# ChenJiahao031008/EAO-Fusion

Hardware: AMD Instinct MI355X
Metric: ORB kpts/s (640x480, 1k feat) + local-BA residuals/s (20 KF x 3k pts) (higher is better)
Workload: dtype u8; 1 GPU; ORBextractor FAST+rBRIEF, 640x480, 8-level pyramid, nFeatures 1000, batch=64 synthetic frames per GPU (BASELINE configs[1]); parallelism=frames sharded per GPU, no data-path collective

## Files before the change

### eao_fusion_amd/csrc/orb.hip

```cpp
#include "orb_internal.h"

using namespace eao::orb;

namespace {

__constant__ __align__(16) signed char c_pattern[1024] = {
#include "orb_pattern.inc"
};

constexpr int kResizeRows = 4;
__device__ __forceinline__ unsigned udot2w(unsigned a, unsigned b) {
    typedef unsigned short us2 __attribute__((ext_vector_type(2)));
    return __builtin_amdgcn_udot2(__builtin_bit_cast(us2, a), __builtin_bit_cast(us2, b), 0u, false);
}

struct ResizeLevel { int w, h, pitch, off; };
struct ResizeArgs {
    ResizeLevel D, S;
    double invX, invY;
    int srcIsInput;
    int pyrFrameBytes;
    int G;
    float invG;
    int frameAffinity;
// ... 985 lines not shown
    const float minZ = A.mb, minD = -3, maxD = A.mbf / minZ;
    const float minU = uL - maxD, maxU = uL - minD;
    float outU = -1.0f, outD = -1.0f;
    int outS = -1;
    if (!(maxU < 0)) {
        const uint4 a0 = A.dl[2 * iL], a1 = A.dl[2 * iL + 1];
        unsigned best = 0xFFFFFFFFu;
        for (int iR = lane; iR < A.nr; iR += 64) {
            const eao_keypoint kr = A.kr[iR];
            const float r = 2.0f * A.scale[kr.octave];
            const int maxr = (int)ceilf(kr.y + r), minr = (int)floorf(kr.y - r);
            if (row < minr || row > maxr) continue;
            if (kr.octave < levelL - 1 || kr.octave > levelL + 1) continue;
            if (!(kr.x >= minU && kr.x <= maxU)) continue;
            const uint4 b0 = A.dr[2 * iR], b1 = A.dr[2 * iR + 1];
            const unsigned d = __popc(a0.x ^ b0.x) + __popc(a0.y ^ b0.y) + __popc(a0.z ^ b0.z) + __popc(a0.w ^ b0.w) +
                               __popc(a1.x ^ b1.x) + __popc(a1.y ^ b1.y) + __popc(a1.z ^ b1.z) + __popc(a1.w ^ b1.w);
            best = min(best, (d << 16) | (unsigned)iR);
        }
        for (int dlt = 32; dlt >= 1; dlt >>= 1) best = min(best, (unsigned)__shfl_xor((int)best, dlt));
        const int bestDist = (int)(best >> 16);
        if (best != 0xFFFFFFFFu && bestDist < refc::TH_HIGH) {
            const int bestIdxR = (int)(best & 0xFFFF);
            const float uR0 = A.kr[bestIdxR].x;
            const float sf = A.invScale[levelL];
            const int suL = (int)roundf(uL * sf), svL = (int)roundf(vL * sf), suR0 = (int)roundf(uR0 * sf);
            const int w = 5, Lw = 5;
            int pl, pr;
            const uint8_t* imgL = level_ptr(g, sl, levelL, A.frame, &pl);
            const uint8_t* imgR = level_ptr(g, sr, levelL, A.frame, &pr);
            const int lw = g->L[levelL].w, lh = g->L[levelL].h;
            const float iniu = (float)(suR0 + Lw - w), endu = (float)(suR0 + Lw + w + 1);
            if (!(iniu < 0 || endu >= (float)lw)) {
                const int cL = px_reflect(imgL, pl, lw, lh, suL, svL);
                int dL0 = 0, dL1 = 0, px0x = 0, px0y = 0, px1x = 0, px1y = 0;
                const bool has1 = lane + 64 < 121;
                px0y = lane / 11; px0x = lane - px0y * 11;
                dL0 = px_reflect(imgL, pl, lw, lh, suL - w + px0x, svL - w + px0y) - cL;
                if (has1) {
                    px1y = (lane + 64) / 11; px1x = lane + 64 - px1y * 11;
                    dL1 = px_reflect(imgL, pl, lw, lh, suL - w + px1x, svL - w + px1y) - cL;
                }
                int dists[11];
                int bestSad = 0x7FFFFFFF, bestinc = 0;
#pragma unroll
                for (int inc = -5; inc <= 5; inc++) {
                    const int cR = px_reflect(imgR, pr, lw, lh, suR0 + inc, svL);
                    int sacc = abs(dL0 - (px_reflect(imgR, pr, lw, lh, suR0 + inc - w + px0x, svL - w + px0y) - cR));
                    if (has1) sacc += abs(dL1 - (px_reflect(imgR, pr, lw, lh, suR0 + inc - w + px1x, svL - w + px1y) - cR));
                    for (int dlt = 32; dlt >= 1; dlt >>= 1) sacc += __shfl_xor(sacc, dlt);
                    dists[inc + 5] = sacc;
                    if (sacc < bestSad) { bestSad = sacc; bestinc = inc; }
                }
                if (!(bestinc == -Lw || bestinc == Lw)) {
                    float dist1 = 0, dist2 = 0, dist3 = 0;
#pragma unroll
                    for (int k = 0; k < 11; k++) {
                        if (k == Lw + bestinc - 1) dist1 = (float)dists[k];
                        if (k == Lw + bestinc) dist2 = (float)dists[k];
                        if (k == Lw + bestinc + 1) dist3 = (float)dists[k];
                    }
                    const float deltaR = (dist1 - dist3) / (2.0f * (dist1 + dist3 - 2.0f * dist2));
                    if (!(deltaR < -1 || deltaR > 1)) {
                        float bestuR = A.scale[levelL] * ((float)suR0 + (float)bestinc + deltaR);
                        float disparity = uL - bestuR;
                        if (disparity >= 0 && disparity < maxD) {
                            if (disparity <= 0) { disparity = 0.01f; bestuR = uL - 0.01f; }
                            outD = A.mbf / disparity;
                            outU = bestuR;
                            outS = bestSad;
                        }
                    }
                }
            }
        }
    }
    if (lane == 0) { A.uRight[iL] = outU; A.depth[iL] = outD; A.sad[iL] = outS; }
}

namespace eao {
namespace orb {

static int blur_mfma_mode() { static const int mode = [] { const char* e = getenv("EAO_ORB_BLUR_MFMA"); return e ? atoi(e) : 1; }(); return mode; }

eao_status enqueue(eao_orb* h, const uint8_t* d_img, int pitch0, long long fs0, int batch, eao_keypoint* d_kps,
                   uint8_t* d_desc, int cap, int* d_n, hipStream_t st) {
    const Geom& g = h->geom;
    eao::Range rAll("eao_orb_extract: enqueue");
    ImgSrc s;
    s.img0 = d_img; s.pitch0 = pitch0; s.fs0 = fs0; s.pyr = h->d_pyr.p;
    h->lastSrc = s; h->lastBatch = batch; h->lastComplete = false; h->pyrFrame = -1;
    const bool prof = h->profiling;
    hipEvent_t* ev = nullptr;
    if (prof) {
        if (h->evUsed + kProfEvents > h->evs.size()) {
            const size_t old = h->evs.size();
            h->evs.resize(old + kProfEvents * 16, nullptr);
            for (size_t i = old; i < h->evs.size(); i++) EAO_HIP(hipEventCreate(&h->evs[i]));
        }
        ev = &h->evs[h->evUsed];
        h->evUsed += kProfEvents;
        EAO_HIP(hipEventRecord(ev[0], st));
    }
    eao_status so;
    if (h->evLastValid && h->lastStream != st) {
        if ((so = order_behind_last_call(h, st))) return so;
    }
    h->lastStream = st;
    EAO_HIP(hipEventRecord(h->evStart, st));
    const hipStream_t ss = h->side;
    const int cells0 = g.L[0].nCells;
    const bool early0 = !prof && g.nlevels > 1 && g.L[0].cellBase == 0 && cells0 < g.totalCells;
    const int aff = (batch & 7) == 0 ? 1 : 0;
    auto fast = [&](hipStream_t str, int first, int end) {
        eao::Range rg("orb: FAST cells");
        const bool whole = first == 0 && end == g.totalCells, narrow = g.fastStride == 48;
        auto* kern = whole ? (narrow ? k_fast_cells<true, 48> : k_fast_cells<true, kTileStrideWide>)
                           : (narrow ? k_fast_cells<false, 48> : k_fast_cells<false, kTileStrideWide>);
        hipLaunchKernelGGL(kern, dim3(128 * ((end - first + 127) / 128), batch), dim3(64), g.fastLdsBytes, str, h->d_geom.p, h->d_cells.p, s,
                           h->d_cellcand.p, h->d_cellcnt.p, 0, first, end, aff);
    };
    const int mid = early0 && batch >= 48 && g.nlevels > 3 ? 3 : 0;
    const bool qtEarly = mid > 0 && batch <= 96;
    const int src0Aligned = ((((uintptr_t)s.img0 | (uintptr_t)s.pitch0 | (uintptr_t)(batch > 1 ? s.fs0 : 0)) & 3) == 0) ? 1 : 0;
    auto quadtree = [&](hipStream_t str, int lFirst, int nLev) {
        eao::Range rg("orb: quad-tree");
        launch_quadtree(h, str, batch, 0, lFirst, nLev);
    };
    auto blur = [&]() -> eao_status {
        EAO_HIP(hipStreamWaitEvent(ss, h->evFork, 0));
        if (prof) EAO_HIP(hipEventRecord(ev[6], ss));
        {
            eao::Range rg("orb: blur");
            if (g.mTotalTiles && blur_mfma_mode())
                hipLaunchKernelGGL(k_blur7_mfma, dim3(g.mTotalTiles, batch), dim3(256), 0, ss, h->d_geom.p, s, h->d_blur.p, h->d_blurTab.p, 0, src0Aligned, aff);
            else hipLaunchKernelGGL(k_blur7, dim3(g.totalTiles, batch), dim3(256), 0, ss, h->d_geom.p, s, h->d_blur.p, 0, src0Aligned, aff);
        }
        if (prof) EAO_HIP(hipEventRecord(ev[7], ss));
        EAO_HIP(hipEventRecord(h->evJoin, ss));
        return EAO_OK;
    };
    auto describe = [&](hipStream_t str, int lFirst, int lEnd, int writeN) {
        eao::Range rg("orb: orientation + description");
        int pairs = 0;
        for (int l = lFirst; l < lEnd; l++) pairs += eao::cdiv(g.L[l].listCap, 2);
        const int gx = std::max(1, eao::cdiv(std::min(pairs, eao::cdiv(cap, 2) + g.nlevels), 4));
        hipLaunchKernelGGL(k_orient_describe, aff ? dim3(8 * gx, batch / 8) : dim3(gx, batch), dim3(256), 0, str,
                           h->d_geom.p, s, h->d_blur.p, h->d_levelkps.p, h->d_levelcnt.p, d_kps, d_desc, d_n, cap, 0, g.nlevels, lFirst, lEnd, writeN, aff);
    };
    if (h->pyrFused && batch <= 32) {
        auto pyramid = [&] {
            eao::Range rg("orb: pyramid");
            hipLaunchKernelGGL(k_pyramid_fused, dim3(h->pyr.tilesX * h->pyr.tilesY, 1, batch), dim3(kPyrThreads), h->pyrLds, st, h->pyr, s, 0);
        };
        if (prof) {
            pyramid();
            EAO_HIP(hipEventRecord(ev[1], st));
            EAO_HIP(hipEventRecord(h->evFork, st));
            if ((so = blur())) return so;
            EAO_HIP(hipStreamWaitEvent(st, h->evJoin, 0));
            EAO_HIP(hipEventRecord(ev[9], st));
            fast(st, 0, g.totalCells);
            EAO_HIP(hipEventRecord(ev[2], st));
            quadtree(st, 0, g.nlevels);
            EAO_HIP(hipEventRecord(ev[3], st));
            EAO_HIP(hipEventRecord(ev[4], st));
        } else {
            EAO_HIP(hipStreamWaitEvent(ss, h->evStart, 0));
            fast(ss, 0, cells0);
            quadtree(ss, 0, 1);
            pyramid();
            EAO_HIP(hipEventRecord(h->evFork, st));
            if ((so = blur())) return so;
            fast(st, cells0, g.totalCells);
            quadtree(st, 1, g.nlevels - 1);
            EAO_HIP(hipStreamWaitEvent(st, h->evJoin, 0));
        }
    } else {
        if (early0) {
            EAO_HIP(hipStreamWaitEvent(ss, h->evStart, 0));
            fast(ss, 0, cells0);
        }
        for (int l = 1; l < g.nlevels; l++) {
            const int G4 = eao::cdiv(g.L[l].w, 4);
            ResizeArgs ra;
            ra.G = G4; ra.invG = 1.0f / (float)G4;
            ra.D = {g.L[l].w, g.L[l].h, g.L[l].pitch, g.L[l].off};
            ra.S = {g.L[l - 1].w, g.L[l - 1].h, g.L[l - 1].pitch, g.L[l - 1].off};
            ra.invX = 1. / ((double)g.L[l].w / g.L[l - 1].w); ra.invY = 1. / ((double)g.L[l].h / g.L[l - 1].h);
            ra.srcIsInput = l == 1; ra.pyrFrameBytes = g.pyrFrameBytes;
            ra.frameAffinity = aff;
            { eao::Range rg("orb: pyramid"); hipLaunchKernelGGL(k_resize, dim3(eao::cdiv(G4 * eao::cdiv(g.L[l].h, kResizeRows), 64), 1, batch), dim3(64), 0, st, ra, s, 0); }
            if (l == mid - 1) {
                EAO_HIP(hipEventRecord(h->evMid, st));
                EAO_HIP(hipStreamWaitEvent(ss, h->evMid, 0));
                fast(ss, cells0, g.L[mid].cellBase);
                if (qtEarly) quadtree(ss, 0, mid);
            }
        }
        if (early0 && !qtEarly) EAO_HIP(hipEventRecord(h->evFast0, ss));
        if (prof) {
            EAO_HIP(hipEventRecord(ev[1], st));
            EAO_HIP(hipEventRecord(h->evFork, st));
            if ((so = blur())) return so;
            EAO_HIP(hipStreamWaitEvent(st, h->evJoin, 0));
            EAO_HIP(hipEventRecord(ev[9], st));
            fast(st, 0, g.totalCells);
            EAO_HIP(hipEventRecord(ev[2], st));
        } else {
            EAO_HIP(hipEventRecord(h->evFork, st));
            fast(st, early0 ? (mid ? g.L[mid].cellBase : cells0) : 0, g.totalCells);
            if ((so = blur())) return so;
            if (early0 && !qtEarly) EAO_HIP(hipStreamWaitEvent(st, h->evFast0, 0));
        }
        quadtree(st, qtEarly ? mid : 0, g.nlevels - (qtEarly ? mid : 0));
        if (prof) EAO_HIP(hipEventRecord(ev[3], st));
        EAO_HIP(hipStreamWaitEvent(st, h->evJoin, 0));
        if (prof) EAO_HIP(hipEventRecord(ev[4], st));
    }
    describe(st, 0, g.nlevels, 1);
    if (prof) {
        EAO_HIP(hipEventRecord(ev[5], st));
        EAO_HIP(hipEventRecord(ev[8], st));
    }
    h->evLastValid = true;
    if (h->everyCallEvent) { EAO_HIP(hipEventRecord(h->evLast, st)); h->evLastRecorded = true; }
    EAO_HIP(hipGetLastError());
    return EAO_OK;
}

__global__ __launch_bounds__(256) void k_stream_download(const uint4* __restrict__ src, uint4* __restrict__ dst, size_t n16) {
    for (size_t i = (size_t)blockIdx.x * 256 + threadIdx.x; i < n16; i += (size_t)gridDim.x * 256) dst[i] = src[i];
}

struct PyrExportLevel { int w, h, srcPitch, srcOff, dstPitch, rowChunks, chunkBase; long long dstOff; };
struct PyrExportArgs { int nlevels, border, totalChunks, pyrFrameBytes; PyrExportLevel L[kMaxLevels]; };
__global__ __launch_bounds__(256) void k_pyramid_export(PyrExportArgs A, ImgSrc s, int frame, uint8_t* __restrict__ dst) {
    const int idx = blockIdx.x * 256 + threadIdx.x;
    if (idx >= A.totalChunks) return;
    int l = 0;
    while (l + 1 < A.nlevels && idx >= A.L[l + 1].chunkBase) l++;
    const PyrExportLevel& L = A.L[l];
    const int r = idx - L.chunkBase, row = r / L.rowChunks, ch = r - row * L.rowChunks;
    const uint8_t* src = l == 0 ? s.img0 + (long long)frame * s.fs0 : s.pyr + (long long)frame * A.pyrFrameBytes + L.srcOff;
    const int pitch = l == 0 ? s.pitch0 : L.srcPitch;
    int y = row - A.border;
    y = y < 0 ? -y : (y >= L.h ? 2 * L.h - 2 - y : y);
    y = min(max(y, 0), L.h - 1);
    const uint8_t* srow = src + (long long)y * pitch;
    unsigned w4[4];
#pragma unroll
    for (int q = 0; q < 4; q++) {
        unsigned v = 0;
#pragma unroll
        for (int b = 0; b < 4; b++) {
            int x = ch * 16 + q * 4 + b - A.border;
            x = x < 0 ? -x : (x >= L.w ? 2 * L.w - 2 - x : x);
            x = min(max(x, 0), L.w - 1);
            v |= (unsigned)srow[x] << (8 * b);
        }
        w4[q] = v;
    }
    *reinterpret_cast<uint4*>(dst + L.dstOff + (long long)row * L.dstPitch + ch * 16) = make_uint4(w4[0], w4[1], w4[2], w4[3]);
}

eao_status enqueue_pyramid_export(eao_orb* h, int frame, int border) {
    const Geom& g = h->geom;
    for (int l = 0; l < g.nlevels; l++) EAO_REQUIRE(border < g.L[l].w && border < g.L[l].h, "level %d is smaller than the border", l);
    PyrExportArgs A;
    A.nlevels = g.nlevels; A.border = border; A.pyrFrameBytes = g.pyrFrameBytes;
    size_t off = 0;
    int chunks = 0;
    for (int l = 0; l < g.nlevels; l++) {
        PyrExportLevel& L = A.L[l];
        L.w = g.L[l].w; L.h = g.L[l].h; L.srcPitch = g.L[l].pitch; L.srcOff = g.L[l].off;
// ... 145 lines not shown
```

### eao_fusion_amd/csrc/orb_host.hip

```cpp
#include "orb_internal.h"

using namespace eao::orb;

namespace eao {
namespace orb {

eao_status build_geometry(eao_orb* h, int W, int H) {
    const eao_orb_cfg& c = h->cfg;
    Geom& g = h->geom;
    std::memset(&g, 0, sizeof(g));
    g.nlevels = c.nlevels; g.W = W; g.H = H;
    g.iniTh = c.ini_th_fast; g.minTh = c.min_th_fast;
    for (int i = 0; i < 16; i++) g.umax[i] = h->umax[i];
    h->cells.clear();
    int off = 0, kpBase = 0, candBase = 0, tileBase = 0, maxCell = 0, scanCap = 0, maxList = 0, maxSw = 0, maxSh = 0;
    for (int l = 0; l < c.nlevels; l++) {
        LevelGeom& L = g.L[l];
        const float s = h->invScale[l];
        L.w = cv_round((float)W * s);
        L.h = cv_round((float)H * s);
        EAO_REQUIRE(L.w < 4096 && L.h < 4096, "level %d is %dx%d: coordinates are packed in 12 bits", l, L.w, L.h);
        const int maxBX = L.w - kEdge + 3, maxBY = L.h - kEdge + 3;
        const float width = (float)(maxBX - kMinBorder), height = (float)(maxBY - kMinBorder);
        const int nCols = (int)(width / (float)refc::FAST_CELL), nRows = (int)(height / (float)refc::FAST_CELL);
// ... 111 lines not shown
            }
            coefCap = (coefCap + 7) & ~3;
            P.coefOff = (int)lds; P.coefCap = coefCap;
            lds += (size_t)coefCap * 16;
            h->pyrLds = lds;
            h->pyrFused = lds <= 64 * 1024 && h->cfg.scale_factor <= 2.0f;
            for (int l = 1; l < c.nlevels; l++)
                if (P.L[l].invX > 2.0 || P.L[l].invY > 2.0) h->pyrFused = false;
            if (h->pyrFused) {
                std::vector<int2> cxv, cyv;
                for (int l = 1; l < c.nlevels; l++) {
                    P.L[l].coefXOff = (int)cxv.size(); P.L[l].coefYOff = (int)cyv.size();
                    for (int d = 0; d < g.L[l].w; d++) { int o; unsigned w2; resize_coef_host(d, P.L[l].invX, g.L[l - 1].w, true, &o, &w2); cxv.push_back(make_int2(o, (int)w2)); }
                    for (int d = 0; d < g.L[l].h; d++) { int o; unsigned w2; resize_coef_host(d, P.L[l].invY, g.L[l - 1].h, false, &o, &w2); cyv.push_back(make_int2(o, (int)w2)); }
                }
                eao_status st2 = h->d_pyrRanges.reserve(table.size());
                if (st2) return st2;
                if ((st2 = h->d_pyrCoef.reserve(cxv.size() + cyv.size()))) return st2;
                EAO_HIP(hipMemcpy(h->d_pyrRanges.p, table.data(), table.size() * sizeof(int4), hipMemcpyHostToDevice));
                EAO_HIP(hipMemcpy(h->d_pyrCoef.p, cxv.data(), cxv.size() * sizeof(int2), hipMemcpyHostToDevice));
                EAO_HIP(hipMemcpy(h->d_pyrCoef.p + cxv.size(), cyv.data(), cyv.size() * sizeof(int2), hipMemcpyHostToDevice));
                P.ranges = h->d_pyrRanges.p;
                P.coefX = h->d_pyrCoef.p; P.coefY = h->d_pyrCoef.p + cxv.size();
            }
        }
    }
    g.scanCap = scanCap;
    g.fastMaxTested = std::max(1, (maxSw - 6) * (maxSh - 6));
    g.fastStride = maxSw + 3 <= 48 ? 48 : kTileStrideWide;
    g.fastTileBytes = ((maxSh * g.fastStride) + 15) & ~15;
    g.fastLdsBytes = g.fastTileBytes + ((2 * g.fastMaxTested + 15) & ~15) + ((((maxSw - 4) * (maxSh - 4)) + 15) & ~15) + 64;
    h->quadLds = (size_t)maxList * (2 * sizeof(short4) + sizeof(int) * kQtNodeInts) + (size_t)scanCap * sizeof(int);
    g.qtNodesGlobal = 0; g.qtNodeFrameBytes = 0;
    if (h->quadLds > 100 * 1024) {
        g.qtNodesGlobal = 1;
        long long noff = 0;
        for (int l = 0; l < c.nlevels; l++) {
            g.L[l].nodeOff = noff;
            noff += (long long)align256((size_t)g.L[l].listCap * (2 * sizeof(short4) + sizeof(int) * kQtNodeInts) + (size_t)scanCap * sizeof(int));
        }
        g.qtNodeFrameBytes = noff;
        h->quadLds = 0;
    }
    h->quadLds = (h->quadLds + 15) & ~(size_t)15;
    g.qtKeysOff = (int)h->quadLds;
    const size_t kQtLdsCand = std::min<size_t>(8192, std::max<size_t>(2048, ((size_t)h->cfg.nfeatures * 4 + 63) & ~(size_t)63));
    g.qtLdsCand = (int)std::min<size_t>(kQtLdsCand, h->quadLds < 76 * 1024 ? (76 * 1024 - h->quadLds) / 6 : 0) & ~7;
    h->quadLds += (size_t)g.qtLdsCand * 6;
    if (g.qtNodesGlobal) { g.qtLdsCand = 0; h->quadLds = 0; }
    {
        float cf[7]; double sum = 0;
        for (int i = 0; i < 7; i++) { double x = i - 3; cf[i] = (float)std::exp(-0.5 / 4.0 * x * x); sum += cf[i]; }
        const int expect[7] = {18, 34, 49, 55, 49, 34, 18};
        for (int i = 0; i < 7; i++)
            if (cv_round((double)(float)(cf[i] * (1. / sum)) * 256.0) != expect[i]) { eao::set_error("gaussian taps mismatch"); return EAO_ERR_INTERNAL; }
    }
    {
        std::vector<BlurMLevelIn> in;
        for (int l = 0; l < c.nlevels; l++) in.push_back({g.L[l].w, g.L[l].h, l == 0 ? (g.L[l].w + 3) & ~3 : g.L[l].pitch});
        const BlurMTables T = blur_m_build(in);
        EAO_REQUIRE(T.maxEntry <= 127, "blur table entry %d does not fit int8", T.maxEntry);
        int mBase = 0, any = 0;
        for (int l = 0; l < c.nlevels; l++) {
            LevelGeom& L = g.L[l];
            const BlurMLevel& M = T.level[l];
            L.mOk = M.ok; L.mTilesX = M.tilesX; L.mBlocksY = M.blocksY; L.mXIdx = M.xIdx; L.mYIdx = M.yIdx;
            const int valu = eao::cdiv(L.tilesX * eao::cdiv(L.h, kBlurRows), kBlurStripsPerWg);
            int walkLen;
            const int mfma = eao::cdiv(M.tilesX * blur_m_walks(M.blocksY, &walkLen), 4);
            L.mTileBase = mBase;
            mBase += !M.ok ? valu : l == 0 ? std::max(valu, mfma) : mfma;
            any |= M.ok;
        }
        g.mTotalTiles = any ? mBase : 0;
        g.mFragOff = (int)((T.idx.size() * sizeof(int) + kBlurMFrag - 1) / kBlurMFrag * kBlurMFrag);
        if (any) {
            std::vector<uint8_t> blob((size_t)g.mFragOff + T.frag.size(), 0);
            std::memcpy(blob.data(), T.idx.data(), T.idx.size() * sizeof(int));
            std::memcpy(blob.data() + g.mFragOff, T.frag.data(), T.frag.size());
            { eao_status st = h->d_blurTab.reserve(blob.size()); if (st) return st; }
            EAO_HIP(hipMemcpy(h->d_blurTab.p, blob.data(), blob.size(), hipMemcpyHostToDevice));
        }
    }
    { eao_status st = h->d_geom.reserve(1); if (st) return st; }
    EAO_HIP(hipMemcpyAsync(h->d_geom.p, &g, sizeof(Geom), hipMemcpyHostToDevice, h->stream));
    { eao_status st = h->d_cells.reserve(h->cells.size()); if (st) return st; }
    EAO_HIP(hipMemcpyAsync(h->d_cells.p, h->cells.data(), h->cells.size() * sizeof(CellDesc), hipMemcpyHostToDevice, h->stream));
    EAO_HIP(eao::wait_latency(h->stream));
    { eao_status sq = quadtree_reserve_lds(h->quadLds); if (sq) return sq; }
    h->geomValid = true;
    h->batchCap = 0;
    return EAO_OK;
}

eao_status ensure(eao_orb* h, int W, int H, int batch, hipStream_t caller) {
    eao_status st = eao::require_device();
    if (st) return st;
    if (!h->stream && batch > 0) {
        int least = 0, greatest = 0, p = 0;
        const bool follow = (uintptr_t)caller != kNoCallerStream && !(getenv("EAO_STREAM_PRIORITY") && !atoi(getenv("EAO_STREAM_PRIORITY"))) &&
                            hipDeviceGetStreamPriorityRange(&least, &greatest) == hipSuccess && least != greatest && hipStreamGetPriority(caller, &p) == hipSuccess;
        (void)hipGetLastError();
        auto make = [&](hipStream_t* q) -> hipError_t {
            if ((uintptr_t)caller == kNoCallerStream) return eao::create_stream(q, eao::StreamClass::Latency);
            if (!follow || p == 0) return hipStreamCreateWithFlags(q, hipStreamNonBlocking);
            return hipStreamCreateWithPriority(q, hipStreamNonBlocking, p);
        };
        EAO_HIP(make(&h->stream));
        EAO_HIP(hipEventCreateWithFlags(&h->evStart, hipEventDisableTiming));
        EAO_HIP(hipEventCreateWithFlags(&h->evLast, hipEventDisableTiming));
        EAO_HIP(make(&h->spacer));
        EAO_HIP(make(&h->side));
        for (hipEvent_t* e : {&h->evFork, &h->evFast0, &h->evMid, &h->evJoin}) EAO_HIP(hipEventCreateWithFlags(e, hipEventDisableTiming));
    }
    if (!h->d_dbg && getenv("EAO_DEBUG_STAMPS")) {
        EAO_HIP(hipMalloc(&h->d_dbg, 16 * kMaxLevels * sizeof(long long)));
        EAO_HIP(hipMemset(h->d_dbg, 0, 16 * kMaxLevels * sizeof(long long)));
    }
    if (!h->geomValid || h->geom.W != W || h->geom.H != H) {
        st = build_geometry(h, W, H);
        if (st) return st;
    }
    if (batch > h->batchCap) {
        const Geom& g = h->geom;
        const size_t B = batch;
#define RES(buf, cnt) do { st = h->buf.reserve(cnt); if (st) return st; } while (0)
        RES(d_pyr, B * g.pyrFrameBytes);
        RES(d_blur, B * g.pyrFrameBytes);
        RES(d_cellcand, B * (size_t)g.totalCells * g.cellCap);
        RES(d_cellcnt, B * g.totalCells);
        RES(d_cand, B * (size_t)g.totalCandCap);
        RES(d_nodeof, B * (size_t)g.totalCandCap);
        if (g.qtNodesGlobal) RES(d_qtnodes, B * (size_t)g.qtNodeFrameBytes);
        RES(d_levelkps, B * (size_t)g.totalKpCap);
        RES(d_levelcnt, B * g.nlevels);
        RES(d_candcnt, B * g.nlevels);
#undef RES
        h->batchCap = batch;
    }
    return EAO_OK;
}

eao_status order_behind_last_call(eao_orb* h, hipStream_t st) {
    if (h->evLastRecorded) EAO_HIP(hipStreamWaitEvent(st, h->evLast, 0));
    else EAO_HIP(hipDeviceSynchronize());
    h->everyCallEvent = true;
    return EAO_OK;
}

void stream_release(eao_orb* h) {
    for (eao_orb::StreamSlot& sl : h->slots) {
        if (sl.evOut && sl.submitted) (void)hipEventSynchronize(sl.evOut);
        if (sl.pinIn) (void)hipHostFree(sl.pinIn);
        if (sl.pinOut) (void)hipHostFree(sl.pinOut);
        if (sl.dIn) (void)hipFree(sl.dIn);
        if (sl.dOut) (void)hipFree(sl.dOut);
        if (sl.evIn) (void)hipEventDestroy(sl.evIn);
        if (sl.evOut) (void)hipEventDestroy(sl.evOut);
        if (sl.evDone) (void)hipEventDestroy(sl.evDone);
    }
    h->slots.clear();
    for (hipStream_t* q : {&h->sUp, &h->sRun, &h->sDown})
        if (*q) { (void)hipStreamSynchronize(*q); (void)hipStreamDestroy(*q); *q = nullptr; }
}

eao_status wait_last_extraction(eao_orb* h) {
// ... 365 lines not shown
```

### eao_fusion_amd/csrc/orb_internal.h

```cpp
#pragma once

#include <algorithm>
#include <atomic>
#include <cmath>
#include <cstdlib>
#include <cstring>
#include <vector>

#include "common.h"
#include "orb_blur_tables.h"


namespace eao {
namespace orb {

constexpr int kMaxLevels = 16;
constexpr int kEdge = refc::EDGE_THRESHOLD;
constexpr int kMinBorder = kEdge - 3;
constexpr int kTile = 72;
constexpr int kTileStrideWide = 80;
constexpr int kMaxIni = 16;
constexpr size_t kPinnedOutMax = 1 << 20;
constexpr int kFastXcdRun = 0;

struct LevelGeom {
    int w, h, pitch, off;
    int cellBase, nCells;
    int quota;
    int nIni, boxH;
    float hX;
    int listCap;
    int kpBase;
    int candBase, candCap;
    int tileBase, tilesX;
    int mOk, mTileBase;
    int mTilesX, mBlocksY;
    int mXIdx, mYIdx;
    long long nodeOff;
    int scaledPatch;
    float scale;
};

struct Geom {
    int nlevels, W, H;
    int totalCells, cellCap;
    int totalKpCap, totalCandCap, totalTiles;
    int mTotalTiles, mFragOff;
    int pyrFrameBytes;
    int iniTh, minTh;
    int scanCap;
    int qtLdsCand, qtKeysOff;
    int qtNodesGlobal;
    long long qtNodeFrameBytes;
    int fastMaxTested, fastTileBytes, fastLdsBytes, fastStride;
    int umax[16];
    LevelGeom L[kMaxLevels];
};

struct CellDesc {
    short level, x0, y0, sw, sh, offX, offY, pad;
};

struct ImgSrc {
    const uint8_t* img0;
    int pitch0;
    long long fs0;
    uint8_t* pyr;
};

__device__ __forceinline__ const uint8_t* level_ptr(const Geom* g, const ImgSrc& s, int l, int f, int* pitch) {
    if (l == 0) {
        *pitch = s.pitch0;
        return s.img0 + (long long)f * s.fs0;
    }
    *pitch = g->L[l].pitch;
    return s.pyr + (long long)f * g->pyrFrameBytes + g->L[l].off;
}

constexpr int kPyrTW = 128, kPyrTH = 32;
constexpr int kPyrThreads = 256;
struct PyrLevel { int w, h, pitch, off; double invX, invY; int ldsOff, ldsW, ldsH; int coefXOff, coefYOff; };
struct PyrArgs {
    int nlevels, tilesX, tilesY, pyrFrameBytes;
    int coefOff;
    int coefCap;
    PyrLevel L[kMaxLevels];
    const int4* ranges;
    const int2* coefX;
    const int2* coefY;
};

constexpr int kQTSmall = 1024, kQTLarge = 256;
constexpr int kQtNodeInts = 2 + 2 + 2 + 4 + 4 + 5;

constexpr size_t kProfEvents = 10;


inline void resize_coef_host(int d, double inv, int slimit, bool clampHi, int* ofs, unsigned* wpair) {
    float fr = (float)(((double)d + 0.5) * inv - 0.5);
    int o = (int)std::floor(fr);
    fr -= (float)o;
    if (clampHi) {
        if (o < 0) { fr = 0; o = 0; }
        if (o >= slimit - 1) { fr = 0; o = slimit - 1; }
    }
    const int w0 = std::min(std::max((int)std::lrintf((1.f - fr) * 2048.f), -32768), 32767);
    const int w1 = std::min(std::max((int)std::lrintf(fr * 2048.f), -32768), 32767);
    *ofs = o;
    *wpair = ((unsigned)w0 & 0xFFFFu) | ((unsigned)w1 << 16);
}

__host__ __device__ inline int pyr_src_ofs(int d, double inv, int sn) {
    float fr = (float)(((double)d + 0.5) * inv - 0.5);
    int o = (int)floorf(fr);
    return o < 0 ? 0 : (o > sn - 1 ? sn - 1 : o);
}
__host__ __device__ inline int pyr_first_at_least(int bound, double inv, int sn, int dn) {
    if (bound <= 0) return 0;
    int d = (int)((double)bound / inv);
    d = d < 0 ? 0 : (d > dn ? dn : d);
    while (d > 0 && pyr_src_ofs(d - 1, inv, sn) >= bound) d--;
    while (d < dn && pyr_src_ofs(d, inv, sn) < bound) d++;
    return d;
}

constexpr int kBlurRows = 16;
constexpr int kBlurSegW = 128;
constexpr int kBlurStripsPerWg = 8;
inline int cv_round(double v) { return (int)std::lrint(v); }

}
}

struct eao_orb {
    using Geom = eao::orb::Geom; using CellDesc = eao::orb::CellDesc; using PyrArgs = eao::orb::PyrArgs; using ImgSrc = eao::orb::ImgSrc;
    eao_orb_cfg cfg;
    std::vector<float> scale, invScale, sigma2, invSigma2;
    std::vector<int> quota;
    int umax[16];
    Geom geom;
    bool geomValid = false;
    int batchCap = 0;
    std::vector<CellDesc> cells;
    size_t quadLds = 0;
    eao::DevBuf<int4> d_pyrRanges;
    eao::DevBuf<int2> d_pyrCoef;
    PyrArgs pyr;
    size_t pyrLds = 0;
    bool pyrFused = false;
    hipStream_t stream = nullptr;
    hipStream_t side = nullptr;
    hipStream_t spacer = nullptr;
    bool evLastValid = false;
    hipStream_t lastStream = nullptr;
    hipEvent_t evLast = nullptr;
    bool everyCallEvent = false, evLastRecorded = false;
    hipEvent_t evStart = nullptr, evFork = nullptr, evJoin = nullptr, evFast0 = nullptr, evMid = nullptr;
    eao::DevBuf<Geom> d_geom;
    eao::DevBuf<CellDesc> d_cells;
    eao::DevBuf<uint8_t> d_pyr, d_blur, d_in;
    eao::DevBuf<uint8_t> d_blurTab;
    eao::DevBuf<unsigned> d_cellcand, d_cand, d_levelkps;
    eao::DevBuf<unsigned short> d_nodeof;
    eao::DevBuf<unsigned char> d_qtnodes;
    eao::DevBuf<int> d_cellcnt, d_levelcnt, d_candcnt, d_nout;
    eao::DevBuf<eao_keypoint> d_kps;
    unsigned char* pinOut = nullptr;
    size_t pinOutCap = 0;
    unsigned char* pinUp = nullptr;
    size_t pinUpCap = 0;
    eao::DevBuf<uint8_t> d_desc;
    eao::DevBuf<float> d_xyr;
    eao::DevBuf<unsigned char> d_stereo;
    unsigned char* pinPyr = nullptr;
    size_t pinPyrCap = 0;
    eao_orb_level_view pyrViews[eao::orb::kMaxLevels] = {};
    int pyrFrame = -1, pyrBorder = -1;
    int autoPyrBorder = -1;
    bool lastComplete = false;
    ImgSrc lastSrc{};
    int lastBatch = 0;
    bool profiling = false;
    long long* d_dbg = nullptr;
    std::vector<hipEvent_t> evs;
    size_t evUsed = 0;
    struct StreamSlot {
        unsigned char* pinIn = nullptr; unsigned char* pinOut = nullptr;
        unsigned char* pinOutDev = nullptr;
        unsigned char* dIn = nullptr; unsigned char* dOut = nullptr;
        hipEvent_t evIn = nullptr, evDone = nullptr, evOut = nullptr;
        int batch = 0;
        bool submitted = false;
    };
    std::vector<StreamSlot> slots;
    hipStream_t sUp = nullptr, sRun = nullptr, sDown = nullptr;
    int sW = 0, sH = 0, sB = 0, sCap = 0, sPitch = 0;
    size_t sInBytes = 0, sOutBytes = 0, sOffK = 0, sOffD = 0;
};

namespace eao {
namespace orb {
constexpr uintptr_t kNoCallerStream = ~(uintptr_t)0;
eao_status ensure(eao_orb* h, int W, int H, int batch, hipStream_t caller = (hipStream_t)kNoCallerStream);
eao_status order_behind_last_call(eao_orb* h, hipStream_t st);
void stream_release(eao_orb* h);
eao_status wait_last_extraction(eao_orb* h);
eao_status upload_frames(eao_orb* h, const uint8_t* img, int width, int height, int stride, long long frame_stride, int batch);
eao_status enqueue(eao_orb* h, const uint8_t* d_img, int pitch0, long long fs0, int batch, eao_keypoint* d_kps, uint8_t* d_desc, int cap, int* d_n, hipStream_t st);
eao_status enqueue_pyramid_export(eao_orb* h, int frame, int border);
void launch_quadtree(const eao_orb* h, hipStream_t str, int nb, int f0, int lFirst, int nLev);
eao_status quadtree_reserve_lds(size_t bytes);
}
}
```

Before: 277.7 million kpts/s.

## Add MFMA int8 matrix-multiply path for pyramid bilinear resize

Adds a new resize kernel that expresses the horizontal bilinear interpolation as int8 MFMA matmuls against precomputed per-tile weight strips, with vertical blending done in registers from LDS-staged source rows. Host code builds deduplicated weight/row tables at geometry setup and uploads them. The enqueue path uses it by default when tables are valid, falling back to the old VALU kernel otherwise. It aims to cut ALU cost of the 7 pyramid resize launches, at the risk of bit-exactness issues from splitting weights into high/low int8 pieces and added per-tile LDS staging.

```diff
diff --git a/eao_fusion_amd/csrc/orb.hip b/eao_fusion_amd/csrc/orb.hip
--- a/eao_fusion_amd/csrc/orb.hip
+++ b/eao_fusion_amd/csrc/orb.hip
@@ -1091,6 +1091,7 @@
 namespace orb {
 
 static int blur_mfma_mode() { static const int mode = [] { const char* e = getenv("EAO_ORB_BLUR_MFMA"); return e ? atoi(e) : 1; }(); return mode; }
+static int resize_mfma_mode() { static const int mode = [] { const char* e = getenv("EAO_ORB_RESIZE_MFMA"); return e ? atoi(e) : 1; }(); return mode; }
 
 eao_status enqueue(eao_orb* h, const uint8_t* d_img, int pitch0, long long fs0, int batch, eao_keypoint* d_kps,
                    uint8_t* d_desc, int cap, int* d_n, hipStream_t st) {
@@ -1199,7 +1200,8 @@
             ra.invX = 1. / ((double)g.L[l].w / g.L[l - 1].w); ra.invY = 1. / ((double)g.L[l].h / g.L[l - 1].h);
             ra.srcIsInput = l == 1; ra.pyrFrameBytes = g.pyrFrameBytes;
             ra.frameAffinity = aff;
-            { eao::Range rg("orb: pyramid"); hipLaunchKernelGGL(k_resize, dim3(eao::cdiv(G4 * eao::cdiv(g.L[l].h, kResizeRows), 64), 1, batch), dim3(64), 0, st, ra, s, 0); }
+            if (h->resizeM[l].ok && (l > 1 || src0Aligned) && resize_mfma_mode()) { eao::Range rg("orb: pyramid"); launch_resize_mfma(h, st, s, l, batch, aff); }
+            else { eao::Range rg("orb: pyramid"); hipLaunchKernelGGL(k_resize, dim3(eao::cdiv(G4 * eao::cdiv(g.L[l].h, kResizeRows), 64), 1, batch), dim3(64), 0, st, ra, s, 0); }
             if (l == mid - 1) {
                 EAO_HIP(hipEventRecord(h->evMid, st));
                 EAO_HIP(hipStreamWaitEvent(ss, h->evMid, 0));
diff --git a/eao_fusion_amd/csrc/orb_host.hip b/eao_fusion_amd/csrc/orb_host.hip
--- a/eao_fusion_amd/csrc/orb_host.hip
+++ b/eao_fusion_amd/csrc/orb_host.hip
@@ -217,6 +217,24 @@
             EAO_HIP(hipMemcpy(h->d_blurTab.p, blob.data(), blob.size(), hipMemcpyHostToDevice));
         }
     }
+    {
+        std::vector<ResizeMLevelIn> in;
+        for (int l = 0; l < c.nlevels; l++) in.push_back({g.L[l].w, g.L[l].h, l == 0 ? (g.L[l].w + 3) & ~3 : g.L[l].pitch});
+        const ResizeMTables T = resize_m_build(in);
+        EAO_REQUIRE(T.maxPiece <= 127, "resize table piece %d does not fit int8", T.maxPiece);
+        int any = 0;
+        for (int l = 0; l < kMaxLevels; l++) { h->resizeM[l] = l < c.nlevels ? T.level[l] : ResizeMLevel{}; any |= h->resizeM[l].ok; }
+        if (any) {
+            h->resizeMRowsOff = (T.idx.size() * sizeof(int) + 15) & ~(size_t)15;
+            h->resizeMStripsOff = h->resizeMRowsOff + T.rows.size() * sizeof(ResizeMRow);
+            std::vector<uint8_t> blob(h->resizeMStripsOff + T.strips.size(), 0);
+            std::memcpy(blob.data(), T.idx.data(), T.idx.size() * sizeof(int));
+            std::memcpy(blob.data() + h->resizeMRowsOff, T.rows.data(), T.rows.size() * sizeof(ResizeMRow));
+            std::memcpy(blob.data() + h->resizeMStripsOff, T.strips.data(), T.strips.size());
+            { eao_status st = h->d_resizeTab.reserve(blob.size()); if (st) return st; }
+            EAO_HIP(hipMemcpy(h->d_resizeTab.p, blob.data(), blob.size(), hipMemcpyHostToDevice));
+        }
+    }
     { eao_status st = h->d_geom.reserve(1); if (st) return st; }
     EAO_HIP(hipMemcpyAsync(h->d_geom.p, &g, sizeof(Geom), hipMemcpyHostToDevice, h->stream));
     { eao_status st = h->d_cells.reserve(h->cells.size()); if (st) return st; }
diff --git a/eao_fusion_amd/csrc/orb_internal.h b/eao_fusion_amd/csrc/orb_internal.h
--- a/eao_fusion_amd/csrc/orb_internal.h
+++ b/eao_fusion_amd/csrc/orb_internal.h
@@ -9,6 +9,7 @@
 
 #include "common.h"
 #include "orb_blur_tables.h"
+#include "orb_resize_tables.h"
 
 
 namespace eao {
@@ -95,20 +96,6 @@
 
 constexpr size_t kProfEvents = 10;
 
-
-inline void resize_coef_host(int d, double inv, int slimit, bool clampHi, int* ofs, unsigned* wpair) {
-    float fr = (float)(((double)d + 0.5) * inv - 0.5);
-    int o = (int)std::floor(fr);
-    fr -= (float)o;
-    if (clampHi) {
-        if (o < 0) { fr = 0; o = 0; }
-        if (o >= slimit - 1) { fr = 0; o = slimit - 1; }
-    }
-    const int w0 = std::min(std::max((int)std::lrintf((1.f - fr) * 2048.f), -32768), 32767);
-    const int w1 = std::min(std::max((int)std::lrintf(fr * 2048.f), -32768), 32767);
-    *ofs = o;
-    *wpair = ((unsigned)w0 & 0xFFFFu) | ((unsigned)w1 << 16);
-}
 
 __host__ __device__ inline int pyr_src_ofs(int d, double inv, int sn) {
     float fr = (float)(((double)d + 0.5) * inv - 0.5);
@@ -160,6 +147,9 @@
     eao::DevBuf<CellDesc> d_cells;
     eao::DevBuf<uint8_t> d_pyr, d_blur, d_in;
     eao::DevBuf<uint8_t> d_blurTab;
+    eao::DevBuf<uint8_t> d_resizeTab;
+    eao::orb::ResizeMLevel resizeM[eao::orb::kMaxLevels] = {};
+    size_t resizeMRowsOff = 0, resizeMStripsOff = 0;
     eao::DevBuf<unsigned> d_cellcand, d_cand, d_levelkps;
     eao::DevBuf<unsigned short> d_nodeof;
     eao::DevBuf<unsigned char> d_qtnodes;
@@ -208,6 +198,7 @@
 eao_status upload_frames(eao_orb* h, const uint8_t* img, int width, int height, int stride, long long frame_stride, int batch);
 eao_status enqueue(eao_orb* h, const uint8_t* d_img, int pitch0, long long fs0, int batch, eao_keypoint* d_kps, uint8_t* d_desc, int cap, int* d_n, hipStream_t st);
 eao_status enqueue_pyramid_export(eao_orb* h, int frame, int border);
+void launch_resize_mfma(const eao_orb* h, hipStream_t str, const ImgSrc& s, int l, int batch, int frameAffinity);
 void launch_quadtree(const eao_orb* h, hipStream_t str, int nb, int f0, int lFirst, int nLev);
 eao_status quadtree_reserve_lds(size_t bytes);
 }
diff --git a/eao_fusion_amd/csrc/orb_resize_mfma.hip b/eao_fusion_amd/csrc/orb_resize_mfma.hip
--- /dev/null
+++ b/eao_fusion_amd/csrc/orb_resize_mfma.hip
@@ -0,0 +1,144 @@
+#include "orb_internal.h"
+
+using namespace eao::orb;
+
+namespace {
+
+typedef int rm_v4i __attribute__((ext_vector_type(4)));
+typedef int rm_v16i __attribute__((ext_vector_type(16)));
+typedef rm_v4i rm_v4i_a4 __attribute__((aligned(4)));
+typedef unsigned short rm_u16x2 __attribute__((ext_vector_type(2)));
+
+constexpr int kLdsPitch = 80;
+constexpr int kLoads = 4;
+static_assert(kResizeMRows == 16 * (kLoads + 1), "a block's rows beyond the prefetched ones are one more load");
+
+struct ResizeMArgs {
+    int dw, dh, dpitch, doff;
+    int sh, spitch, soff;
+    int srcIsInput, pyrFrameBytes;
+    int tilesX, blocksY, walkLen;
+    int frameAffinity;
+};
+
+__device__ __forceinline__ void rm_load(const uint8_t* __restrict__ src, int spitch, int sh, int base, int n, unsigned ws, int lane, rm_v4i raw[kLoads]) {
+#pragma unroll
+    for (int k = 0; k < kLoads; k++)
+        if (k < n) {
+            const int y = min(base + 16 * k + (lane >> 2), sh - 1);
+            raw[k] = *reinterpret_cast<const rm_v4i_a4*>(src + (unsigned)(__umul24(y, spitch) + ws + 16 * (lane & 3)));
+        }
+}
+
+__global__ __launch_bounds__(64, 4) void k_resize_mfma(ResizeMArgs A, ImgSrc s, int f0, const int2* __restrict__ idx, const int4* __restrict__ rows,
+                                                    const uint8_t* __restrict__ strips) {
+    int f = blockIdx.z, bx = blockIdx.x;
+    if (A.frameAffinity) {
+        const unsigned b = blockIdx.x + gridDim.x * blockIdx.z, xcd = b & 7, slot = b >> 3;
+        f = (int)(xcd + 8 * (slot / gridDim.x)); bx = (int)(slot % gridDim.x);
+    }
+    f += f0;
+    const int lane = threadIdx.x, half = lane >> 5;
+    const int cx = bx % A.tilesX, b0 = (bx / A.tilesX) * A.walkLen;
+    const int b1 = min(b0 + A.walkLen, A.blocksY);
+    if (b0 >= b1) return;
+    const int spitch = A.srcIsInput ? s.pitch0 : A.spitch;
+    const uint8_t* src = A.srcIsInput ? s.img0 + (long long)f * s.fs0 : s.pyr + (long long)f * A.pyrFrameBytes + A.soff;
+    uint8_t* dst = s.pyr + (long long)f * A.pyrFrameBytes + A.doff;
+    const int2 xi = idx[cx];
+    const unsigned ws = (unsigned)xi.x;
+    const uint8_t* tab = strips + xi.y;
+    const rm_v4i t10 = *reinterpret_cast<const rm_v4i*>(tab + lane * 16), t11 = *reinterpret_cast<const rm_v4i*>(tab + kResizeMFrag + lane * 16);
+    const rm_v4i t00 = *reinterpret_cast<const rm_v4i*>(tab + 2 * kResizeMFrag + lane * 16), t01 = *reinterpret_cast<const rm_v4i*>(tab + 3 * kResizeMFrag + lane * 16);
+    rm_v16i coff;
+#pragma unroll
+    for (int q = 0; q < 4; q++) {
+        const rm_v4i o = *reinterpret_cast<const rm_v4i*>(tab + 4 * kResizeMFrag + 4 * (8 * q + 4 * half));
+#pragma unroll
+        for (int e = 0; e < 4; e++) coff[4 * q + e] = o[e];
+    }
+    asm volatile("" : "+v"(coff));
+    rm_v16i z;
+#pragma unroll
+    for (int q = 0; q < 16; q++) z[q] = 0;
+    __shared__ __attribute__((aligned(16))) uint8_t stage[kResizeMRows * kLdsPitch];
+    const rm_v4i bias = {(int)0x80808080u, (int)0x80808080u, (int)0x80808080u, (int)0x80808080u};
+
+    rm_v4i raw[kLoads];
+    int base = rows[kResizeMTile * b0].x;
+    int n = (rows[kResizeMTile * b0 + kResizeMTile - 1].y - base + 16) >> 4;
+    int4 rt = rows[kResizeMTile * b0 + (lane & 31)];
+    rm_load(src, spitch, A.sh, base, n, ws, lane, raw);
+    for (int b = b0; b < b1; b++) {
+        eao::wave_sync();
+#pragma unroll
+        for (int k = 0; k < kLoads; k++)
+            if (k < n) *reinterpret_cast<rm_v4i*>(stage + (16 * k + (lane >> 2)) * kLdsPitch + 16 * (lane & 3)) = raw[k] ^ bias;
+        if (n > kLoads) {
+            const int y = min(base + 16 * kLoads + (lane >> 2), A.sh - 1);
+            const rm_v4i late = *reinterpret_cast<const rm_v4i_a4*>(src + (unsigned)(__umul24(y, spitch) + ws + 16 * (lane & 3)));
+            *reinterpret_cast<rm_v4i*>(stage + (16 * kLoads + (lane >> 2)) * kLdsPitch + 16 * (lane & 3)) = late ^ bias;
+        }
+        eao::wave_sync();
+        const uint8_t* p0 = stage + (rt.x - base) * kLdsPitch + 16 * half;
+        const uint8_t* p1 = stage + (rt.y - base) * kLdsPitch + 16 * half;
+        const rm_v4i a00 = *reinterpret_cast<const rm_v4i*>(p0), a01 = *reinterpret_cast<const rm_v4i*>(p0 + 32);
+        const rm_v4i a10 = *reinterpret_cast<const rm_v4i*>(p1), a11 = *reinterpret_cast<const rm_v4i*>(p1 + 32);
+        const unsigned B0 = (unsigned)rt.z << 16, B1 = (unsigned)rt.w << 16;
+        if (b + 1 < b1) {
+            base = rows[kResizeMTile * (b + 1)].x;
+            n = (rows[kResizeMTile * (b + 1) + kResizeMTile - 1].y - base + 16) >> 4;
+            rt = rows[kResizeMTile * (b + 1) + (lane & 31)];
+            rm_load(src, spitch, A.sh, base, n, ws, lane, raw);
+        }
+        rm_v16i h0 = __builtin_amdgcn_mfma_i32_32x32x32_i8(t10, a00, z, 0, 0, 0);
+        rm_v16i l0 = __builtin_amdgcn_mfma_i32_32x32x32_i8(t00, a00, coff, 0, 0, 0);
+        rm_v16i h1 = __builtin_amdgcn_mfma_i32_32x32x32_i8(t10, a10, z, 0, 0, 0);
+        rm_v16i l1 = __builtin_amdgcn_mfma_i32_32x32x32_i8(t00, a10, coff, 0, 0, 0);
+        h0 = __builtin_amdgcn_mfma_i32_32x32x32_i8(t11, a01, h0, 0, 0, 0);
+        l0 = __builtin_amdgcn_mfma_i32_32x32x32_i8(t01, a01, l0, 0, 0, 0);
+        h1 = __builtin_amdgcn_mfma_i32_32x32x32_i8(t11, a11, h1, 0, 0, 0);
+        l1 = __builtin_amdgcn_mfma_i32_32x32x32_i8(t01, a11, l1, 0, 0, 0);
+        unsigned o[4];
+#pragma unroll
+        for (int q = 0; q < 4; q++) {
+            unsigned sv[4];
+#pragma unroll
+            for (int e = 0; e < 4; e++) {
+                const unsigned H0 = ((unsigned)h0[4 * q + e] << 6) + (unsigned)l0[4 * q + e], H1 = ((unsigned)h1[4 * q + e] << 6) + (unsigned)l1[4 * q + e];
+                sv[e] = __umulhi(B0, H0 >> 4) + __umulhi(B1, H1 >> 4) + 2;
+            }
+            const rm_u16x2 two = {2, 2};
+            const rm_u16x2 pa = __builtin_bit_cast(rm_u16x2, sv[0] | (sv[1] << 16)) >> two, pb = __builtin_bit_cast(rm_u16x2, sv[2] | (sv[3] << 16)) >> two;
+            o[q] = __builtin_amdgcn_perm(__builtin_bit_cast(unsigned, pb), __builtin_bit_cast(unsigned, pa), 0x06040200u);
+        }
+        const auto s02 = __builtin_amdgcn_permlane32_swap(o[0], o[2], false, false);
+        const auto s13 = __builtin_amdgcn_permlane32_swap(o[1], o[3], false, false);
+        const int y = kResizeMTile * b + (lane & 31);
+        if (y < A.dh) *reinterpret_cast<uint4*>(dst + (unsigned)(__umul24(y, A.dpitch) + kResizeMTile * cx + 16 * half)) = make_uint4(s02[0], s02[1], s13[0], s13[1]);
+    }
+}
+
+}
+
+namespace eao {
+namespace orb {
+
+void launch_resize_mfma(const eao_orb* h, hipStream_t str, const ImgSrc& s, int l, int batch, int frameAffinity) {
+    const Geom& g = h->geom;
+    const ResizeMLevel& M = h->resizeM[l];
+    ResizeMArgs A;
+    A.dw = g.L[l].w; A.dh = g.L[l].h; A.dpitch = g.L[l].pitch; A.doff = g.L[l].off;
+    A.sh = g.L[l - 1].h; A.spitch = g.L[l - 1].pitch; A.soff = g.L[l - 1].off;
+    A.srcIsInput = l == 1; A.pyrFrameBytes = g.pyrFrameBytes;
+    A.tilesX = M.tilesX; A.blocksY = M.blocksY;
+    const int walks = resize_m_walks(M.blocksY, &A.walkLen);
+    A.frameAffinity = frameAffinity;
+    const int2* idx = reinterpret_cast<const int2*>(h->d_resizeTab.p) + M.xIdx;
+    const int4* rows = reinterpret_cast<const int4*>(h->d_resizeTab.p + h->resizeMRowsOff) + M.rowOff;
+    const uint8_t* strips = h->d_resizeTab.p + h->resizeMStripsOff;
+    hipLaunchKernelGGL(k_resize_mfma, dim3(M.tilesX * walks, 1, batch), dim3(64), 0, str, A, s, 0, idx, rows, strips);
+}
+
+}
+}
diff --git a/eao_fusion_amd/csrc/orb_resize_tables.h b/eao_fusion_amd/csrc/orb_resize_tables.h
--- /dev/null
+++ b/eao_fusion_amd/csrc/orb_resize_tables.h
@@ -0,0 +1,162 @@
+#pragma once
+
+#include <algorithm>
+#include <cmath>
+#include <cstdint>
+#include <cstring>
+#include <map>
+#include <string>
+#include <vector>
+
+namespace eao {
+namespace orb {
+
+constexpr int kResizeMTile = 32;
+constexpr int kResizeMWin = 64;
+constexpr int kResizeMSeg = 4;
+constexpr int kResizeMFrag = 1024;
+constexpr int kResizeMRows = 80;
+constexpr int kResizeMStrip = 4 * kResizeMFrag + 4 * kResizeMTile;
+
+inline void resize_coef_host(int d, double inv, int slimit, bool clampHi, int* ofs, unsigned* wpair) {
+    float fr = (float)(((double)d + 0.5) * inv - 0.5);
+    int o = (int)std::floor(fr);
+    fr -= (float)o;
+    if (clampHi) {
+        if (o < 0) { fr = 0; o = 0; }
+        if (o >= slimit - 1) { fr = 0; o = slimit - 1; }
+    }
+    const int w0 = std::min(std::max((int)std::lrintf((1.f - fr) * 2048.f), -32768), 32767);
+    const int w1 = std::min(std::max((int)std::lrintf(fr * 2048.f), -32768), 32767);
+    *ofs = o;
+    *wpair = ((unsigned)w0 & 0xFFFFu) | ((unsigned)w1 << 16);
+}
+
+struct ResizeMLevelIn { int w, h, readable; };
+struct ResizeMLevel {
+    int ok;
+    int tilesX, blocksY;
+    int xIdx;
+    int rowOff;
+    int maxSpan;
+};
+struct ResizeMRow { int sy0, sy1, b0, b1; };
+struct ResizeMTables {
+    std::vector<ResizeMLevel> level;
+    std::vector<int> idx;
+    std::vector<ResizeMRow> rows;
+    std::vector<uint8_t> strips;
+    int maxPiece = 0;
+};
+
+#if defined(__HIPCC__)
+__host__ __device__
+#endif
+inline int resize_m_walks(int blocksY, int* len) {
+    const int n = (blocksY + kResizeMSeg - 1) / kResizeMSeg;
+    *len = (blocksY + n - 1) / n;
+    return n;
+}
+
+inline bool resize_m_strip(int cx, int dw, int sw, int readable, double invX, int* wsOut, uint8_t* out , int* maxPiece) {
+    int comb[kResizeMTile][2][2];
+    int lo = 1 << 30, hi = -1;
+    for (int c = 0; c < kResizeMTile; c++) {
+        const int x = kResizeMTile * cx + c;
+        comb[c][0][1] = comb[c][1][1] = 0; comb[c][0][0] = comb[c][1][0] = 0;
+        if (x >= dw) continue;
+        int o; unsigned wp;
+        resize_coef_host(x, invX, sw, true, &o, &wp);
+        const int w0 = (short)(wp & 0xFFFF), w1 = (short)(wp >> 16);
+        if (w0 < 0 || w1 < 0) return false;
+        comb[c][0][0] = o; comb[c][0][1] = w0;
+        comb[c][1][0] = std::min(o + 1, sw - 1); comb[c][1][1] = w1;
+        for (int t = 0; t < 2; t++)
+            if (comb[c][t][1]) { lo = std::min(lo, comb[c][t][0]); hi = std::max(hi, comb[c][t][0]); }
+    }
+    if (hi < 0) return false;
+    int ws = lo & ~15;
+    if (ws > readable - kResizeMWin) ws = readable - kResizeMWin;
+    if (ws < 0 || (ws & 3) || lo < ws || hi >= ws + kResizeMWin) return false;
+    *wsOut = ws;
+    std::memset(out, 0, kResizeMStrip);
+    int weight[kResizeMTile][kResizeMWin] = {};
+    int32_t colOff[kResizeMTile];
+    for (int c = 0; c < kResizeMTile; c++) {
+        int sum = 0;
+        for (int t = 0; t < 2; t++)
+            if (comb[c][t][1]) { weight[c][comb[c][t][0] - ws] += comb[c][t][1]; sum += comb[c][t][1]; }
+        colOff[c] = 128 * sum;
+        for (int k = 0; k < kResizeMWin; k++) {
+            const int c1 = weight[c][k] >> 6, c0 = weight[c][k] & 63;
+            if (c1 > 127) return false;
+            *maxPiece = std::max(*maxPiece, std::max(c1, c0));
+            const int slot = (c + 32 * ((k >> 4) & 1)) * 16 + (k & 15);
+            out[(0 + (k >> 5)) * kResizeMFrag + slot] = (uint8_t)c1;
+            out[(2 + (k >> 5)) * kResizeMFrag + slot] = (uint8_t)c0;
+        }
+    }
+    std::memcpy(out + 4 * kResizeMFrag, colOff, sizeof(colOff));
+    return true;
+}
+
+inline ResizeMTables resize_m_build(const std::vector<ResizeMLevelIn>& in) {
+    ResizeMTables T;
+    std::map<std::string, int> seen;
+    std::vector<uint8_t> buf(kResizeMStrip);
+    for (size_t l = 0; l < in.size(); l++) {
+        ResizeMLevel M{};
+        if (l == 0) { T.level.push_back(M); continue; }
+        const ResizeMLevelIn &D = in[l], &S = in[l - 1];
+        M.tilesX = (D.w + kResizeMTile - 1) / kResizeMTile;
+        M.blocksY = (D.h + kResizeMTile - 1) / kResizeMTile;
+        M.ok = D.w > 0 && D.h > 0 && S.w > 0 && S.h > 0 && S.readable >= S.w && S.readable >= kResizeMWin && (S.readable & 3) == 0;
+        const double invX = 1. / ((double)D.w / S.w), invY = 1. / ((double)D.h / S.h);
+        std::vector<int> idx;
+        std::vector<std::string> fresh;
+        std::map<std::string, int> mine;
+        for (int cx = 0; M.ok && cx < M.tilesX; cx++) {
+            int ws = 0;
+            if (!resize_m_strip(cx, D.w, S.w, S.readable, invX, &ws, buf.data(), &T.maxPiece)) { M.ok = 0; break; }
+            const std::string key((const char*)buf.data(), buf.size());
+            int off;
+            auto it = seen.find(key);
+            if (it != seen.end()) off = it->second;
+            else if ((it = mine.find(key)) != mine.end()) off = it->second;
+            else {
+                off = (int)(T.strips.size() + fresh.size() * kResizeMStrip);
+                mine.emplace(key, off);
+                fresh.push_back(key);
+            }
+            idx.push_back(ws); idx.push_back(off);
+        }
+        std::vector<ResizeMRow> rows;
+        for (int y = 0; M.ok && y < kResizeMTile * M.blocksY; y++) {
+            int o; unsigned wp;
+            resize_coef_host(std::min(y, D.h - 1), invY, S.h, false, &o, &wp);
+            ResizeMRow R;
+            R.sy0 = std::min(std::max(o, 0), S.h - 1); R.sy1 = std::min(std::max(o + 1, 0), S.h - 1);
+            R.b0 = (short)(wp & 0xFFFF); R.b1 = (short)(wp >> 16);
+            if (R.b0 < 0 || R.b1 < 0) M.ok = 0;
+            if (!rows.empty() && (R.sy0 < rows.back().sy0 || R.sy1 < rows.back().sy1)) M.ok = 0;
+            rows.push_back(R);
+        }
+        for (int b = 0; M.ok && b < M.blocksY; b++) {
+            const int span = rows[kResizeMTile * b + kResizeMTile - 1].sy1 - rows[kResizeMTile * b].sy0 + 1;
+            if (span > kResizeMRows) M.ok = 0;
+            M.maxSpan = std::max(M.maxSpan, span);
+        }
+        if (M.ok) {
+            M.xIdx = (int)T.idx.size() / 2; M.rowOff = (int)T.rows.size();
+            T.idx.insert(T.idx.end(), idx.begin(), idx.end());
+            T.rows.insert(T.rows.end(), rows.begin(), rows.end());
+            for (const std::string& k : fresh) T.strips.insert(T.strips.end(), k.begin(), k.end());
+            seen.insert(mine.begin(), mine.end());
+        } else M.maxSpan = 0;
+        T.level.push_back(M);
+    }
+    return T;
+}
+
+}
+}
```

Result: faster. 286.3 million kpts/s (median of 6 runs) (+3.1%).
